# kumar-shridhar/PyTorch-BayesianCNN

Measured on AMD Instinct MI355X. Metric: MC-forward samples/sec, BayesianAlexNet CIFAR-10 bs=512 num_ens=10, higher is better.
Workload: dtype f32; 1 GPU; BayesianAlexNet 3x32x32 -> 10, layer_type=bbb, softplus, bs=512, num_ens=10, forward only; global_batch=512, num_ens_total=10, parallelism=single, launch=hipGraph replay, 2 lane(s) x 4 steps per launch

## Files before the change

include/bbb_hip.h:

```cpp
#ifndef BBB_HIP_H
#define BBB_HIP_H

#include <stdint.h>

#ifdef __cplusplus
extern "C" {
#endif

#define BBB_ABI_VERSION 13
#define BBB_MAX_SEGMENTS 16

#define BBB_EINVAL (-1)
#define BBB_EALIGN (-2)
#define BBB_ESHAPE (-3)

typedef struct bbb_segment {
    const float* mu;
    const float* rho;
    float* w;
    float* sigma;
    const float* eps;
    int64_t n;
    int64_t draw_stride;
    uint32_t stream_id;
// ... 28 lines not shown
    int64_t n;
} bbb_adam_segment_t;

int bbb_adam_step(const bbb_adam_segment_t* segs, int nseg, double lr, double beta1, double beta2, double eps,
                  int64_t step, const float* step_dev, const float* lr_dev, void* stream);

int bbb_eps_dump(float* out, int64_t n, int64_t start, uint64_t seed, uint32_t call, uint32_t stream_id, void* stream);

typedef struct bbb_conv_desc {
    int32_t batch;
    int32_t cin, h, w;
    int32_t cout, kh, kw;
    int32_t stride_h, stride_w, pad_h, pad_w, dil_h, dil_w;
    int32_t draws;
    int64_t x_draw_stride;
    int64_t w_draw_stride;
    int64_t b_draw_stride;
    int32_t act;
    int32_t unit_div;
    int32_t unit_off;
    int32_t x_unit_mod;
    int32_t w_row_pitch;
    int32_t b_offset;
    int32_t x_unit_div;
    int32_t x_unit_off;
    int32_t pool;
    int32_t w_tap_major;
} bbb_conv_desc_t;

int bbb_conv2d_fwd(const bbb_conv_desc_t* d, const float* x, const float* w, const float* bias,
                   float* y, void* stream);

int bbb_lrt_conv2d_fwd(const bbb_conv_desc_t* d, const float* x, const float* w_mu, const float* w_var,
                       const float* b_mu, const float* b_var, float* y,
                       float* act_mu_out, float* act_var_out, const float* eps_ext,
                       uint64_t seed, uint32_t call0, uint32_t stream_id, int sample,
                       const uint32_t* call_dev, void* stream);

int bbb_conv2d_chwn_fwd(const bbb_conv_desc_t* d, const float* x, const float* w, const float* bias,
                        float* y, void* stream);
#define BBB_S3_IN  1u
#define BBB_S3_OUT 2u
int bbb_conv2d_chwn_bf16x3_fwd(const bbb_conv_desc_t* d, const void* x, const float* w, const float* bias, void* y, uint32_t flags,
                               void* stream);
int bbb_maxpool_chwn_s3(const void* x, void* y, int64_t slabs, int channels, int h, int w, int batch, int k, int s, void* stream);
int bbb_s3_convert(const void* src, void* dst, int64_t slabs, int64_t n, int to_s3, void* stream);
#define BBB_C8X3_OUT_F32 1u
#define BBB_C8X3_TILE128 2u
#define BBB_C8X3_TILE256 4u
#define BBB_C8X3_POOL 8u
#define BBB_C8X3_NT_SHIFT 4
#define BBB_C8X3_NT_MASK 0x70u
#define BBB_C8X3_ZERO_LEAD_H(n) (((uint32_t)(n) & 15u) << 8)
#define BBB_C8X3_ZERO_LEAD_W(n) (((uint32_t)(n) & 15u) << 12)
#define BBB_C8X3_ZERO_TRAIL_H(n) (((uint32_t)(n) & 15u) << 16)
#define BBB_C8X3_ZERO_TRAIL_W(n) (((uint32_t)(n) & 15u) << 20)
#define BBB_C8X3_ZERO_MASK 0x00FFFF00u
int bbb_conv2d_c8x3_fwd(const bbb_conv_desc_t* d, const void* x, const float* w, const float* bias, void* y, uint32_t flags,
                        void* stream);
int bbb_c8s3_convert(const void* src, void* dst, int64_t slabs, int channels, int64_t positions, int batch, int to_c8s3, void* stream);
int bbb_lrt_conv2d_c8x3_fwd(const bbb_conv_desc_t* d, const void* x, const float* w_mu, const float* w_var, const float* b_mu,
                            const float* b_var, void* y, uint64_t seed, uint32_t call0, uint32_t stream_id, int sample,
                            const uint32_t* call_dev, uint32_t flags, void* stream);
int bbb_maxpool_chwn_s3sq(const void* x, void* y, int64_t slabs, int channels, int h, int w, int batch, int k, int s, void* stream);
int bbb_s2d_c8s3sq(const float* x, void* y, int64_t blocks, int batch, int channels, int h, int w, int k, int stride, int pad, void* stream);
int bbb_s2d_c8s3(const float* x, void* y, int64_t blocks, int batch, int channels, int h, int w, int k, int stride, int pad, void* stream);
int bbb_w_s2d_tap_major(const float* w, float* out, int64_t rows, int channels, int k, int stride, void* stream);
int bbb_w_tap_major(const float* w, float* out, int64_t rows, int cin, int taps, void* stream);
int bbb_lrt_conv2d_chwn_fwd(const bbb_conv_desc_t* d, const float* x, const float* w_mu, const float* w_var,
                            const float* b_mu, const float* b_var, float* y,
                            float* act_mu_out, float* act_var_out, const float* eps_ext,
                            uint64_t seed, uint32_t call0, uint32_t stream_id, int sample,
                            const uint32_t* call_dev, void* stream);

int64_t bbb_conv2d_chwn_splitk_scratch(const bbb_conv_desc_t* d, int lrt, int32_t* k_split);
int bbb_conv2d_chwn_splitk_fwd(const bbb_conv_desc_t* d, const float* x, const float* w, const float* bias, float* y,
                               int k_split, void* scratch, int64_t scratch_bytes, void* stream);
int bbb_lrt_conv2d_chwn_splitk_fwd(const bbb_conv_desc_t* d, const float* x, const float* w_mu, const float* w_var,
                                   const float* b_mu, const float* b_var, float* y,
                                   float* act_mu_out, float* act_var_out, const float* eps_ext,
                                   uint64_t seed, uint32_t call0, uint32_t stream_id, int sample,
                                   const uint32_t* call_dev, int k_split, void* scratch, int64_t scratch_bytes, void* stream);

int bbb_maxpool_chwn(const float* x, float* y, int64_t planes, int h, int w, int batch, int k, int s, void* stream);

int bbb_pool_act_bwd_chwn(const float* g_out, const float* y, float* g_pre, int64_t planes, int h, int w, int batch,
                          int k, int s, int act, int64_t out_plane_pitch, void* stream);

int bbb_lrt_pool_act_bwd_chwn(const float* g_out, const float* y, const float* act_mu, const float* act_var, float* g_mu,
                              float* g_var, int64_t planes, int64_t moment_planes, int h, int w, int batch, int k, int s, int act,
                              int64_t out_plane_pitch, const float* g_out2, const float* x_out, int64_t x_planes, void* stream);

int bbb_lrt_sample_chwn(const float* act_mu, const float* act_var, float* y, int draws, int channels, int pixels, int batch,
                        int b_offset, int act, uint64_t seed, uint32_t call0, uint32_t stream_id, const uint32_t* call_dev,
                        void* stream);

int bbb_lrt_sample_nchw(const float* act_mu, const float* act_var, float* y, int64_t n, int draws, uint64_t seed,
                        uint32_t call0, uint32_t stream_id, const uint32_t* call_dev, void* stream);

#define BBB_BF16_OUT_F32      1u
#define BBB_BF16_W_TAP_MAJOR  2u
#define BBB_BF16_X_C8         4u
#define BBB_BF16_OUT_C8       8u
int bbb_conv2d_chwn_bf16_fwd(const bbb_conv_desc_t* d, const void* x, const void* w, const float* bias, void* y,
                             uint32_t flags, void* stream);
int bbb_maxpool_chwn_bf16(const void* x, void* y, int64_t planes, int h, int w, int batch, int k, int s, void* stream);
int bbb_nchw_to_chwn_bf16(const float* x, void* y, int batch, int64_t plane, void* stream);
int bbb_nchw_to_chwn_bf16_slices(const float* x, void* y, int batch, int64_t plane, int slices, void* stream);

int bbb_mc_tail(const float* logits, int draws, int batch, int classes, int mean_over,
                float* lse_out, void* stream);

int bbb_mc_tail_cb(const float* logits, int draws, int batch, int classes, int mean_over,
                   float* lse_out, void* stream);
int bbb_mc_tail_cb_bwd(const float* logits, const float* lse, const float* g_lse, float* g_logits, int draws, int batch, int classes,
                       int mean_over, void* stream);

int bbb_elbo_cb_fwd(const float* lse, const int64_t* target, const float* kl, float beta, const float* beta_dev, float train_size,
                    int batch, int classes, float* loss_out, void* stream);
int bbb_elbo_cb_bwd(const float* logits, const float* lse, const int64_t* target, const float* g_loss, float beta,
                    const float* beta_dev, float train_size, float* g_logits, float* g_kl, int draws, int batch, int classes,
                    int mean_over, void* stream);

int bbb_mc_tail_units(const float* logits, int units, int slices, int unit_off, int batch_slice, int classes, int mean_over,
                      float* lse_out, void* stream);

int bbb_mc_tail_units_step(const float* logits, int units, int slices, int unit_off, int batch_slice, int classes, int mean_over,
                           float* lse_out, const float* kl_in, float kl_scale, float* kl_out, uint32_t* counter,
                           uint32_t counter_add, void* stream);

int bbb_mc_tail_groups_step(const float* logits, int groups, int draws, int batch, int classes, int mean_over,
                            float* lse_out, const float* kl_in, float kl_scale, float* kl_out, uint32_t* counter,
                            uint32_t counter_add, void* stream);

int bbb_mc_tail_share_step(const float* logits, int slabs, int steps, int draws, int first_off, int batch, int classes,
                           float* lse_out, const float* kl_in, float kl_scale, float* kl_out, uint32_t* counter,
                           uint32_t counter_add, void* stream);

int bbb_uncertainty(const float* logits, int draws, int batch, int classes, int normalized,
                    float* pred, float* epistemic, float* aleatoric, void* stream);

int bbb_transpose2d(const float* in, float* out, int64_t rows, int64_t cols, void* stream);

int bbb_transpose_batched(const float* in, float* out, int rows, int cols, int nb1, int nb2, int64_t in_b1, int64_t in_b2,
                          int64_t in_row, int64_t out_b1, int64_t out_b2, int64_t out_col, void* stream);

int bbb_transpose_sum_batched(const float* in, float* out, int rows, int cols, const int32_t* nb, const int64_t* in_b,
                              const int64_t* out_b, int64_t in_row, int64_t out_col, int nsum, int64_t in_sum, int64_t square_off,
                              void* stream);

int bbb_flip_transpose_w(const float* w, float* out, int64_t draws, int cout, int cin, int khkw, void* stream);
int bbb_flip_transpose_w_pair(const float* w0, const float* w1, float* out, int64_t draws_each, int cout, int cin, int khkw,
                              void* stream);
typedef struct {
    const float* w0;
    const float* w1;
    float* out;
    int64_t draws;
    int32_t cout, cin, khkw, reserved;
} bbb_flip_seg_t;
int bbb_flip_transpose_w_multi(const bbb_flip_seg_t* segs, int n_segs, void* stream);

int bbb_im2col_pbj(const float* x, float* out, const bbb_conv_desc_t* d, void* stream);

int bbb_plane_sum(const float* x, float* out, int64_t outer, int64_t rows, int64_t cols, int64_t row_pitch, int64_t outer_stride,
                  void* stream);
// ... 11 lines not shown
```

pytorch-bayesiancnn_amd/bbb_hip/_lib.py:

```python
import ctypes
import os

import torch

_HERE = os.path.dirname(os.path.abspath(__file__))
LIB_PATH = os.environ.get("BBB_HIP_LIB") or os.path.join(_HERE, "libbbb_hip.so")

ABI_VERSION = 13
MAX_SEGMENTS = 16
SIGMA_SQUARED = 1
KL_TEXTBOOK = 2
GW_MEAN_ONLY = 4

c_void_p, c_int, c_float = ctypes.c_void_p, ctypes.c_int, ctypes.c_float
c_u64, c_u32, c_i64, c_i32 = ctypes.c_uint64, ctypes.c_uint32, ctypes.c_int64, ctypes.c_int32


class Segment(ctypes.Structure):
    _fields_ = [("mu", c_void_p), ("rho", c_void_p), ("w", c_void_p), ("sigma", c_void_p), ("eps", c_void_p),
                ("n", c_i64), ("draw_stride", c_i64), ("stream_id", c_u32), ("w_row_len", c_u32), ("w_taps", c_u32), ("w_tm_cin", c_u32)]


class AdamSegment(ctypes.Structure):
    _fields_ = [("param", c_void_p), ("grad", c_void_p), ("exp_avg", c_void_p), ("exp_avg_sq", c_void_p), ("n", c_i64)]


class FlipSeg(ctypes.Structure):
    _fields_ = [("w0", c_void_p), ("w1", c_void_p), ("out", c_void_p), ("draws", c_i64), ("cout", c_i32), ("cin", c_i32),
                ("khkw", c_i32), ("reserved", c_i32)]


class ConvDesc(ctypes.Structure):
    _fields_ = [("batch", c_i32), ("cin", c_i32), ("h", c_i32), ("w", c_i32), ("cout", c_i32), ("kh", c_i32),
                ("kw", c_i32), ("stride_h", c_i32), ("stride_w", c_i32), ("pad_h", c_i32), ("pad_w", c_i32),
                ("dil_h", c_i32), ("dil_w", c_i32), ("draws", c_i32), ("x_draw_stride", c_i64),
                ("w_draw_stride", c_i64), ("b_draw_stride", c_i64), ("act", c_i32),
                ("unit_div", c_i32), ("unit_off", c_i32), ("x_unit_mod", c_i32), ("w_row_pitch", c_i32), ("b_offset", c_i32),
                ("x_unit_div", c_i32), ("x_unit_off", c_i32), ("pool", c_i32), ("w_tap_major", c_i32)]


_SIGNATURES = {
    "bbb_reparam_kl_fwd": (c_int, [ctypes.POINTER(Segment), c_int, c_int, c_float, c_float, c_u64, c_u32, c_u32,
                                   c_void_p, c_void_p, c_void_p, c_void_p, c_void_p]),
    "bbb_reparam_partials": (c_i64, [ctypes.POINTER(Segment), c_int]),
    "bbb_reparam_kl_bwd": (c_int, [ctypes.POINTER(Segment), c_int, c_int, c_float, c_float, c_u64, c_u32, c_u32,
                                   c_void_p, ctypes.POINTER(c_void_p), ctypes.POINTER(c_void_p), c_void_p, c_void_p]),
    "bbb_adam_step": (c_int, [ctypes.POINTER(AdamSegment), c_int, ctypes.c_double, ctypes.c_double, ctypes.c_double, ctypes.c_double,
                            c_i64, c_void_p, c_void_p, c_void_p]),
    "bbb_eps_dump": (c_int, [c_void_p, c_i64, c_i64, c_u64, c_u32, c_u32, c_void_p]),
    "bbb_conv2d_fwd": (c_int, [ctypes.POINTER(ConvDesc), c_void_p, c_void_p, c_void_p, c_void_p, c_void_p]),
    "bbb_lrt_conv2d_fwd": (c_int, [ctypes.POINTER(ConvDesc), c_void_p, c_void_p, c_void_p, c_void_p, c_void_p, c_void_p,
                                   c_void_p, c_void_p, c_void_p, c_u64, c_u32, c_u32, c_int, c_void_p, c_void_p]),
    "bbb_conv2d_chwn_fwd": (c_int, [ctypes.POINTER(ConvDesc), c_void_p, c_void_p, c_void_p, c_void_p, c_void_p]),
    "bbb_conv2d_chwn_bf16x3_fwd": (c_int, [ctypes.POINTER(ConvDesc), c_void_p, c_void_p, c_void_p, c_void_p, c_u32, c_void_p]),
    "bbb_maxpool_chwn_s3": (c_int, [c_void_p, c_void_p, c_i64, c_int, c_int, c_int, c_int, c_int, c_int, c_void_p]),
    "bbb_s3_convert": (c_int, [c_void_p, c_void_p, c_i64, c_i64, c_int, c_void_p]),
    "bbb_conv2d_c8x3_fwd": (c_int, [ctypes.POINTER(ConvDesc), c_void_p, c_void_p, c_void_p, c_void_p, c_u32, c_void_p]),
    "bbb_c8s3_convert": (c_int, [c_void_p, c_void_p, c_i64, c_int, c_i64, c_int, c_int, c_void_p]),
    "bbb_w_tap_major": (c_int, [c_void_p, c_void_p, c_i64, c_int, c_int, c_void_p]),
    "bbb_s2d_c8s3": (c_int, [c_void_p, c_void_p, c_i64, c_int, c_int, c_int, c_int, c_int, c_int, c_int, c_void_p]),
    "bbb_s2d_c8s3sq": (c_int, [c_void_p, c_void_p, c_i64, c_int, c_int, c_int, c_int, c_int, c_int, c_int, c_void_p]),
    "bbb_lrt_conv2d_c8x3_fwd": (c_int, [ctypes.POINTER(ConvDesc), c_void_p, c_void_p, c_void_p, c_void_p, c_void_p, c_void_p, c_u64, c_u32,
                                        c_u32, c_int, c_void_p, c_u32, c_void_p]),
    "bbb_maxpool_chwn_s3sq": (c_int, [c_void_p, c_void_p, c_i64, c_int, c_int, c_int, c_int, c_int, c_int, c_void_p]),
    "bbb_w_s2d_tap_major": (c_int, [c_void_p, c_void_p, c_i64, c_int, c_int, c_int, c_void_p]),
    "bbb_lrt_conv2d_chwn_fwd": (c_int, [ctypes.POINTER(ConvDesc), c_void_p, c_void_p, c_void_p, c_void_p, c_void_p, c_void_p,
                                        c_void_p, c_void_p, c_void_p, c_u64, c_u32, c_u32, c_int, c_void_p, c_void_p]),
    "bbb_lrt_sample_chwn": (c_int, [c_void_p, c_void_p, c_void_p, c_int, c_int, c_int, c_int, c_int, c_int, c_u64, c_u32, c_u32, c_void_p,
                                  c_void_p]),
    "bbb_lrt_sample_nchw": (c_int, [c_void_p, c_void_p, c_void_p, c_i64, c_int, c_u64, c_u32, c_u32, c_void_p, c_void_p]),
    "bbb_maxpool_chwn": (c_int, [c_void_p, c_void_p, c_i64, c_int, c_int, c_int, c_int, c_int, c_void_p]),
    "bbb_pool_act_bwd_chwn": (c_int, [c_void_p, c_void_p, c_void_p, c_i64, c_int, c_int, c_int, c_int, c_int, c_int, c_i64, c_void_p]),
    "bbb_lrt_pool_act_bwd_chwn": (c_int, [c_void_p, c_void_p, c_void_p, c_void_p, c_void_p, c_void_p, c_i64, c_i64, c_int, c_int, c_int,
                                          c_int, c_int, c_int, c_i64, c_void_p, c_void_p, c_i64, c_void_p]),
    "bbb_conv2d_chwn_bf16_fwd": (c_int, [ctypes.POINTER(ConvDesc), c_void_p, c_void_p, c_void_p, c_void_p, c_u32, c_void_p]),
    "bbb_maxpool_chwn_bf16": (c_int, [c_void_p, c_void_p, c_i64, c_int, c_int, c_int, c_int, c_int, c_void_p]),
    "bbb_nchw_to_chwn_bf16": (c_int, [c_void_p, c_void_p, c_int, c_i64, c_void_p]),
    "bbb_nchw_to_chwn_bf16_slices": (c_int, [c_void_p, c_void_p, c_int, c_i64, c_int, c_void_p]),
    "bbb_mc_tail": (c_int, [c_void_p, c_int, c_int, c_int, c_int, c_void_p, c_void_p]),
    "bbb_mc_tail_cb": (c_int, [c_void_p, c_int, c_int, c_int, c_int, c_void_p, c_void_p]),
    "bbb_mc_tail_cb_bwd": (c_int, [c_void_p, c_void_p, c_void_p, c_void_p, c_int, c_int, c_int, c_int, c_void_p]),
    "bbb_mc_tail_units": (c_int, [c_void_p, c_int, c_int, c_int, c_int, c_int, c_int, c_void_p, c_void_p]),
    "bbb_mc_tail_units_step": (c_int, [c_void_p, c_int, c_int, c_int, c_int, c_int, c_int, c_void_p, c_void_p, c_float, c_void_p, c_void_p,
                                       c_u32, c_void_p]),
    "bbb_mc_tail_groups_step": (c_int, [c_void_p, c_int, c_int, c_int, c_int, c_int, c_void_p, c_void_p, c_float, c_void_p, c_void_p,
                                        c_u32, c_void_p]),
    "bbb_mc_tail_share_step": (c_int, [c_void_p, c_int, c_int, c_int, c_int, c_int, c_int, c_void_p, c_void_p, c_float, c_void_p, c_void_p,
                                       c_u32, c_void_p]),
    "bbb_uncertainty": (c_int, [c_void_p, c_int, c_int, c_int, c_int, c_void_p, c_void_p, c_void_p, c_void_p]),
    "bbb_transpose2d": (c_int, [c_void_p, c_void_p, c_i64, c_i64, c_void_p]),
    "bbb_flip_transpose_w": (c_int, [c_void_p, c_void_p, c_i64, c_int, c_int, c_int, c_void_p]),
    "bbb_flip_transpose_w_multi": (c_int, [ctypes.POINTER(FlipSeg), c_int, c_void_p]),
    "bbb_flip_transpose_w_pair": (c_int, [c_void_p, c_void_p, c_void_p, c_i64, c_int, c_int, c_int, c_void_p]),
    "bbb_elbo_cb_fwd": (c_int, [c_void_p, c_void_p, c_void_p, ctypes.c_float, c_void_p, ctypes.c_float, c_int, c_int, c_void_p, c_void_p]),
    "bbb_elbo_cb_bwd": (c_int, [c_void_p, c_void_p, c_void_p, c_void_p, ctypes.c_float, c_void_p, ctypes.c_float, c_void_p, c_void_p,
                                c_int, c_int, c_int, c_int, c_void_p]),
    "bbb_im2col_pbj": (c_int, [c_void_p, c_void_p, ctypes.POINTER(ConvDesc), c_void_p]),
    "bbb_transpose_batched": (c_int, [c_void_p, c_void_p, c_int, c_int, c_int, c_int, c_i64, c_i64, c_i64, c_i64, c_i64, c_i64, c_void_p]),
    "bbb_transpose_sum_batched": (c_int, [c_void_p, c_void_p, c_int, c_int, ctypes.POINTER(c_i32), ctypes.POINTER(c_i64),
                                          ctypes.POINTER(c_i64), c_i64, c_i64, c_int, c_i64, c_i64, c_void_p]),
    "bbb_conv2d_chwn_splitk_scratch": (c_i64, [ctypes.POINTER(ConvDesc), c_int, ctypes.POINTER(c_i32)]),
    "bbb_conv2d_chwn_splitk_fwd": (c_int, [ctypes.POINTER(ConvDesc), c_void_p, c_void_p, c_void_p, c_void_p, c_int, c_void_p, c_i64,
                                           c_void_p]),
    "bbb_lrt_conv2d_chwn_splitk_fwd": (c_int, [ctypes.POINTER(ConvDesc), c_void_p, c_void_p, c_void_p, c_void_p, c_void_p, c_void_p,
                                               c_void_p, c_void_p, c_void_p, c_u64, c_u32, c_u32, c_int, c_void_p, c_int, c_void_p, c_i64,
                                               c_void_p]),
    "bbb_plane_sum": (c_int, [c_void_p, c_void_p, c_i64, c_i64, c_i64, c_i64, c_i64, c_void_p]),
    "bbb_sum_leading": (c_int, [c_void_p, c_void_p, c_i64, c_i64, c_void_p]),
    "bbb_lrt_glue": (c_int, [c_void_p, c_void_p, c_void_p, c_void_p, c_i64, c_i64, c_int, c_void_p]),
    "bbb_abi_version": (c_int, []),
    "bbb_build_info": (ctypes.c_char_p, []),
}
EXPORTS = tuple(_SIGNATURES)

_lib = None


class BBBHipError(RuntimeError):
    pass


def lib():
    global _lib
    if _lib is None:
        if not os.path.exists(LIB_PATH):
            raise BBBHipError(
                f"{LIB_PATH} not found: the HIP kernels are not built. Run ./build.sh "
                "(or `python -c 'import __graft_entry__ as g; g.build()'`). There is no CPU fallback.")
        h = ctypes.CDLL(LIB_PATH)
        for name, (res, args) in _SIGNATURES.items():
            fn = getattr(h, name)
            fn.restype = res
            fn.argtypes = args
        if h.bbb_abi_version() != ABI_VERSION:
            raise BBBHipError(f"ABI mismatch: library reports {h.bbb_abi_version()}, binding expects {ABI_VERSION}")
        _lib = h
    return _lib


_ERR = {-1: "BBB_EINVAL (bad argument)", -2: "BBB_EALIGN (pointer not 4-byte aligned)", -3: "BBB_ESHAPE (bad geometry)"}


def check(rc, what):
    if rc != 0:
        raise BBBHipError(f"{what} failed: {_ERR.get(rc, 'hipError_t %d' % rc)}")


def ptr(t):
    return 0 if t is None else t.data_ptr()


def require_device(*tensors, dtype=torch.float32):
    for t in tensors:
        if t is None:
            continue
        if not t.is_cuda:
            raise BBBHipError("bbb_hip computes on an MI355X only (tensor is on %s); there is no CPU path. "
                              "Move the module / input to 'cuda'." % t.device)
        if t.dtype != dtype:
            raise BBBHipError(f"bbb_hip expects {dtype} tensors here, got {t.dtype}")


_raw_stream = getattr(torch._C, "_cuda_getCurrentRawStream", None)


def cur_stream(device):
    if _raw_stream is not None and device.index is not None:
        return _raw_stream(device.index)
    return torch.cuda.current_stream(device).cuda_stream


class _NoGuard:
    def __enter__(self):
        return self

    def __exit__(self, *exc):
        return False


_NO_GUARD = _NoGuard()


def on_device(device):
    if device.index is None or torch.cuda.current_device() == device.index:
        return _NO_GUARD
    return torch.cuda.device(device)
```

pytorch-bayesiancnn_amd/bbb_hip/ops.py:

```python
import contextlib
import ctypes
import os
import itertools
import sys
import threading
import types
import weakref

import torch

from . import _lib, rng
from ._lib import Segment, ConvDesc, check, ptr, require_device, cur_stream, on_device

_scratch = {}
_retired = []


_scope_tls = threading.local()
_scope_ids = itertools.count(1)


class scratch_scope:

    def __init__(self, owner=None, token=None):
# ... 148 lines not shown

def _desc(x, w, stride, padding, dilation, draws, x_shared, w_shared, act):
    d = ConvDesc()
    Ex, B, Cin, H, W = x.shape
    Ew, Cout, Cin2, kh, kw = w.shape
    if Cin != Cin2:
        raise _lib.BBBHipError(f"channel mismatch: input has {Cin}, weight expects {Cin2}")
    sh, sw = _pair(stride)
    ph, pw = _pair(padding)
    dh, dw = _pair(dilation)
    d.batch, d.cin, d.h, d.w, d.cout, d.kh, d.kw = B, Cin, H, W, Cout, kh, kw
    d.stride_h, d.stride_w, d.pad_h, d.pad_w, d.dil_h, d.dil_w = sh, sw, ph, pw, dh, dw
    d.draws = draws
    d.x_draw_stride = 0 if x_shared else B * Cin * H * W
    d.w_draw_stride = 0 if w_shared else Cout * Cin * kh * kw
    d.b_draw_stride = 0 if w_shared else Cout
    d.act = ACT_CODE[act]
    ho = (H + 2 * ph - dh * (kh - 1) - 1) // sh + 1
    wo = (W + 2 * pw - dw * (kw - 1) - 1) // sw + 1
    return d, ho, wo


def conv2d_forward(x, w, bias, stride=1, padding=0, dilation=1, act=None):
    require_device(x, w, bias)
    x, w = x.contiguous(), w.contiguous()
    bias = None if bias is None else bias.contiguous()
    E = max(x.shape[0], w.shape[0])
    if x.shape[0] not in (1, E) or w.shape[0] not in (1, E):
        raise _lib.BBBHipError("leading (draw) dims of x and w must be 1 or equal")
    d, ho, wo = _desc(x, w, stride, padding, dilation, E, x.shape[0] == 1 and E > 1, w.shape[0] == 1 and E > 1, act)
    y = torch.empty((E, x.shape[1], w.shape[1], ho, wo), dtype=torch.float32, device=x.device)
    with on_device(x.device):
        check(_lib.lib().bbb_conv2d_fwd(ctypes.byref(d), x.data_ptr(), w.data_ptr(), ptr(bias), y.data_ptr(),
                                        cur_stream(x.device)), "bbb_conv2d_fwd")
    return y


def lrt_conv2d_forward(x, w_mu, w_var, b_mu, b_var, seed, call0, stream_id, stride=1, padding=0, dilation=1,
                       sample=True, eps=None, want_moments=False, act=None):
    require_device(x, w_mu, w_var, b_mu, b_var, eps)
    x = x.contiguous()
    w_mu, w_var = w_mu.contiguous(), w_var.contiguous()
    b_mu = None if b_mu is None else b_mu.contiguous()
    b_var = None if b_var is None else b_var.contiguous()
    E = x.shape[0]
    d, ho, wo = _desc(x, w_mu.unsqueeze(0), stride, padding, dilation, E, False, True, act)
    d.w_draw_stride = 0
    d.b_draw_stride = 0
    shape = (E, x.shape[1], w_mu.shape[0], ho, wo)
    y = torch.empty(shape, dtype=torch.float32, device=x.device)
    am = torch.empty(shape, dtype=torch.float32, device=x.device) if want_moments else None
    av = torch.empty(shape, dtype=torch.float32, device=x.device) if want_moments else None
    if eps is not None:
        eps = eps.contiguous()
        if eps.numel() != y.numel():
            raise _lib.BBBHipError("external eps must have the output's shape")
    with on_device(x.device):
        check(_lib.lib().bbb_lrt_conv2d_fwd(ctypes.byref(d), x.data_ptr(), w_mu.data_ptr(), w_var.data_ptr(), ptr(b_mu),
                                            ptr(b_var), y.data_ptr(), ptr(am), ptr(av), ptr(eps), seed,
                                            call0 & 0xFFFFFFFF, stream_id, 1 if sample else 0, rng.call_dev_ptr(x.device),
                                            cur_stream(x.device)),
              "bbb_lrt_conv2d_fwd")
    return y, am, av


@contextlib.contextmanager
def graph_capture(graph, stream=None):
    import gc
    gc.collect()
    was = gc.isenabled()
    gc.disable()
    try:
        with torch.cuda.graph(graph, stream=stream, capture_error_mode="thread_local"):
            yield
    finally:
        if was:
            gc.enable()


class LaunchConfig:
    FIELDS = ("gemm_mode", "bf16x3_min_workgroups", "s3_min_images", "split_k", "pool_fusion", "pool_fuse_min_items",
              "pool_fuse_imbalance", "launches_overlap", "pool_fuse_min_items_overlapped", "pool_fuse_weight_budget",
              "bf16_pool_fuse_min_rows", "bf16_pool_fuse_min_rows_overlapped", "bf16_c8", "bf16_c8_min_items", "c8x3", "c8x3_s2d",
              "dropin_precision")
    __slots__ = FIELDS

    def __init__(self, **kw):
        self.gemm_mode = "fp32"
        self.bf16x3_min_workgroups = 256
        self.s3_min_images = 2048
        self.split_k = True
        self.pool_fusion = True
        self.pool_fuse_min_items = 1536
        self.pool_fuse_imbalance = 1.07
        self.launches_overlap = False
        self.pool_fuse_min_items_overlapped = 400
        self.pool_fuse_weight_budget = 1 << 20
        self.bf16_pool_fuse_min_rows = 0
        self.bf16_pool_fuse_min_rows_overlapped = 0
        self.bf16_c8 = True
        self.bf16_c8_min_items = 0
        self.dropin_precision = "fp32"
        self.c8x3 = True
        self.c8x3_s2d = True
        for k, v in kw.items():
            setattr(self, k, v)

    def copy(self, **kw):
        c = LaunchConfig(**{k: getattr(self, k) for k in self.FIELDS})
        for k, v in kw.items():
            setattr(c, k, v)
        return c

    def key(self):
        return tuple(getattr(self, k) for k in self.FIELDS)

    def __repr__(self):
        return "LaunchConfig(%s)" % ", ".join("%s=%r" % (k, getattr(self, k)) for k in self.FIELDS)


_default_config = LaunchConfig()
_tls = threading.local()


def current_config():
    st = getattr(_tls, "stack", None)
    return st[-1] if st else _default_config


class use_config:

    def __init__(self, cfg=None, **fields):
        self.cfg, self.fields = cfg, fields

    def __enter__(self):
        base = self.cfg if self.cfg is not None else current_config()
        cfg = base.copy(**self.fields) if self.fields else base
        st = getattr(_tls, "stack", None)
        if st is None:
            st = _tls.stack = []
        st.append(cfg)
        return cfg

    def __exit__(self, *a):
        _tls.stack.pop()
        return False


_split_plans = {}


def _split_scratch(d, lrt, device):
    if not current_config().split_k:
        return 1, None
    pkey = (bytes(d), bool(lrt))
    plan = _split_plans.get(pkey)
    if plan is None:
        ks = ctypes.c_int32(1)
        need = _lib.lib().bbb_conv2d_chwn_splitk_scratch(ctypes.byref(d), 1 if lrt else 0, ctypes.byref(ks))
        plan = _split_plans[pkey] = (ks.value, int(need))
    ks_v, need = plan
    if ks_v <= 1:
        return 1, None
    if need <= 0:
        return ks_v, None
    buf = _grow(_scratch_key(device, "splitk"), max(int(need), 1 << 22),
                lambda m: torch.zeros(m, dtype=torch.uint8, device=device))
    return ks_v, buf


def _apply_units(d, units, x_per_slice):
    if units is None:
        return
    S, off = int(units[0]), int(units[1])
    if S > 1:
        d.unit_div, d.unit_off = S, off % S
        d.x_unit_mod = S if x_per_slice else 0


def _desc_chwn(x, w, stride, padding, dilation, draws, x_shared, w_shared, act):
    Ex, Cin, H, W, B = x.shape
    d, ho, wo = _desc(_Shape((Ex, B, Cin, H, W)), w, stride, padding, dilation, draws, x_shared, w_shared, act)
    d.x_draw_stride = 0 if x_shared else Cin * H * W * B
    return d, ho, wo


class overlapped_launches(use_config):

    def __init__(self, on=True):
        super().__init__(launches_overlap=bool(on))


def pool_fusion_ok(x_shape, w_shape, stride, padding, dilation, draws, pool_module=None, fp32_kernel=False):
    cfg = current_config()
    if not cfg.pool_fusion or (cfg.gemm_mode != "fp32" and not fp32_kernel):
        return False
    key = (tuple(x_shape[-4:]), tuple(w_shape[-4:]), _pair(stride), _pair(padding), _pair(dilation), int(draws), cfg.launches_overlap,
           cfg.pool_fuse_min_items, cfg.pool_fuse_imbalance, cfg.pool_fuse_min_items_overlapped, cfg.pool_fuse_weight_budget,
           None if pool_module is None else (str(pool_module.kernel_size), str(pool_module.stride), str(pool_module.padding),
                                             str(pool_module.dilation), pool_module.ceil_mode,
                                             getattr(pool_module, "return_indices", False)))
    hit = _pool_rule_cache.get(key)
    if hit is None:
        if len(_pool_rule_cache) > 512:
            _pool_rule_cache.clear()
        hit = _pool_rule_cache[key] = _pool_fusion_rule(x_shape, w_shape, stride, padding, dilation, draws, pool_module)
    return hit


_pool_rule_cache = {}


def is_pool_2x2(pool_module):
    pr = lambda v: (v, v) if isinstance(v, int) else tuple(v)
    return not (pr(pool_module.kernel_size) != (2, 2) or pr(pool_module.stride if pool_module.stride is not None else 2) != (2, 2) or
                pr(pool_module.padding) != (0, 0) or pr(pool_module.dilation) != (1, 1) or pool_module.ceil_mode or
                getattr(pool_module, "return_indices", False))


def _pool_fusion_rule(x_shape, w_shape, stride, padding, dilation, draws, pool_module):
    cfg = current_config()
    if pool_module is not None and not is_pool_2x2(pool_module):
        return False
    B = x_shape[-1]
    xm = torch.empty((1,) + tuple(x_shape[-4:]), device="meta")
    wm = torch.empty((1,) + tuple(w_shape[-4:]), device="meta")
    d, ho, wo = _desc_chwn(xm, wm, stride, padding, dilation, int(draws), False, False, None)
    if ho % 2 or wo % 2 or B % 4:
        return False
    ks = ctypes.c_int32(1)
    _lib.lib().bbb_conv2d_chwn_splitk_scratch(ctypes.byref(d), 0, ctypes.byref(ks))
    if ks.value > 1:
        return False
    per_group = (ho // 2) * (wo // 2) * -(-B // 128)
    if max(1, 128 // per_group) * 64 * w_shape[-3] * w_shape[-2] * w_shape[-1] * 4 > cfg.pool_fuse_weight_budget:
        return False
    items = int(draws) * per_group * -(-w_shape[-4] // 64)
    if cfg.launches_overlap:
        return items >= cfg.pool_fuse_min_items_overlapped
    return items >= cfg.pool_fuse_min_items and -(-items // 256) * 256 <= cfg.pool_fuse_imbalance * items


def conv2d_chwn_forward(x, w, bias, stride=1, padding=0, dilation=1, act=None, out=None, units=None, n_units=None,
                        x_per_slice=False, x_div=1, bf16x3=None, x_s3=False, out_s3=False, x_off=0, pool=False, w_tap_major=False):
    require_device(w, bias)
    require_device(x, dtype=torch.bfloat16 if x_s3 else torch.float32)
    x, w = x.contiguous(), w.contiguous()
    bias = None if bias is None else bias.contiguous()
    w_mem = w
    if w_tap_major:
        if x_s3 or out_s3 or bf16x3:
            raise _lib.BBBHipError("w_tap_major: fp32 kernel only")
        bf16x3 = False
        w = _Shape((w.shape[0], w.shape[1], w.shape[4], w.shape[2], w.shape[3]))
    if x_s3:
        if x.dim() != 6 or x.shape[1] != 3 or x.shape[5] % 8:
            raise _lib.BBBHipError("an S3 input is a bf16 tensor [E|1, 3, C, H, W, B] with B % 8 == 0")
        x5 = _Shape((x.shape[0],) + tuple(x.shape[2:]))
    else:
        x5 = x
    if units is not None and units[0] > 1:
        E = int(n_units)
        if x5.shape[0] != (units[0] if x_per_slice else E):
            raise _lib.BBBHipError("work units: x must hold one slab per unit, or one per batch slice with x_per_slice")
        d, ho, wo = _desc_chwn(x5, w, stride, padding, dilation, E, False, False, act)
        _apply_units(d, units, x_per_slice)
    elif int(x_div) > 1:
        E = w.shape[0]
        if not 0 <= int(x_off) < int(x_div) or x5.shape[0] != -(-(E + int(x_off)) // int(x_div)):
            raise _lib.BBBHipError("x_div: x must hold ceil((E + x_off) / x_div) input slabs for the E weight sets")
        d, ho, wo = _desc_chwn(x5, w, stride, padding, dilation, E, False, False, act)
        d.x_unit_div, d.x_unit_off = int(x_div), int(x_off)
    else:
        E = max(x5.shape[0], w.shape[0])
        if x5.shape[0] not in (1, E) or w.shape[0] not in (1, E):
            raise _lib.BBBHipError("leading (draw) dims of x and w must be 1 or equal")
        d, ho, wo = _desc_chwn(x5, w, stride, padding, dilation, E, x5.shape[0] == 1 and E > 1, w.shape[0] == 1 and E > 1, act)
    if x_s3:
        d.x_draw_stride *= 3
    if w_tap_major:
        d.w_tap_major = 1
    B = x5.shape[4]
    if pool:
        if x_s3 or out_s3 or bf16x3 or ho % 2 or wo % 2:
            raise _lib.BBBHipError("pool=True: fp32 kernel only, even output height and width")
        d.pool = 1
        ho, wo = ho // 2, wo // 2
    shape = (E, 3, w.shape[1], ho, wo, B) if out_s3 else (E, w.shape[1], ho, wo, B)
    odt = torch.bfloat16 if out_s3 else torch.float32
    if out_s3 and B % 8:
        raise _lib.BBBHipError("an S3 output needs B % 8 == 0")
    if out is None:
        y = torch.empty(shape, dtype=odt, device=x.device)
    else:
        if out.numel() != E * (3 if out_s3 else 1) * w.shape[1] * ho * wo * B or not out.is_contiguous() or out.dtype != odt:
            raise _lib.BBBHipError("out= must be a contiguous tensor of the output's size and dtype")
        y = out.view(shape)
    with on_device(x.device):
        if x_s3 or out_s3 or (not pool and (bf16x3 if bf16x3 is not None else current_config().gemm_mode == "bf16x3")
                              and E * ho * wo * -(-w.shape[1] // 64) * -(-B // 128) >= current_config().bf16x3_min_workgroups):
            check(_lib.lib().bbb_conv2d_chwn_bf16x3_fwd(ctypes.byref(d), x.data_ptr(), w_mem.data_ptr(), ptr(bias), y.data_ptr(),
                                                        (1 if x_s3 else 0) | (2 if out_s3 else 0), cur_stream(x.device)),
                  "bbb_conv2d_chwn_bf16x3_fwd")
            return y
        ks, scr = _split_scratch(d, False, x.device)
        if ks > 1 and pool:
            raise _lib.BBBHipError("pool=True: this layer's contraction is split (conv + maxpool_chwn instead)")
        if ks > 1:
            check(_lib.lib().bbb_conv2d_chwn_splitk_fwd(ctypes.byref(d), x.data_ptr(), w_mem.data_ptr(), ptr(bias), y.data_ptr(), ks,
                                                        ptr(scr), 0 if scr is None else scr.numel(), cur_stream(x.device)),
                  "bbb_conv2d_chwn_splitk_fwd")
        else:
            check(_lib.lib().bbb_conv2d_chwn_fwd(ctypes.byref(d), x.data_ptr(), w_mem.data_ptr(), ptr(bias), y.data_ptr(),
                                                 cur_stream(x.device)), "bbb_conv2d_chwn_fwd")
    return y


def s3_from_f32(x):
    require_device(x)
    x = x.contiguous()
    n = x.numel() // x.shape[0]
    y = torch.empty((x.shape[0], 3) + tuple(x.shape[1:]), dtype=torch.bfloat16, device=x.device)
    with on_device(x.device):
        check(_lib.lib().bbb_s3_convert(x.data_ptr(), y.data_ptr(), x.shape[0], n, 1, cur_stream(x.device)), "bbb_s3_convert")
    return y


def s3_to_f32(x):
    require_device(x, dtype=torch.bfloat16)
    x = x.contiguous()
    n = x.numel() // (3 * x.shape[0])
    y = torch.empty((x.shape[0],) + tuple(x.shape[2:]), dtype=torch.float32, device=x.device)
    with on_device(x.device):
        check(_lib.lib().bbb_s3_convert(x.data_ptr(), y.data_ptr(), x.shape[0], n, 0, cur_stream(x.device)), "bbb_s3_convert")
    return y


def maxpool_chwn_s3(x, k, s):
    require_device(x, dtype=torch.bfloat16)
    x = x.contiguous()
    E, three, C, H, W, B = x.shape
    ho, wo = (H - k) // s + 1, (W - k) // s + 1
    y = torch.empty((E, 3, C, ho, wo, B), dtype=torch.bfloat16, device=x.device)
    with on_device(x.device):
        check(_lib.lib().bbb_maxpool_chwn_s3(x.data_ptr(), y.data_ptr(), E, C, H, W, B, int(k), int(s), cur_stream(x.device)),
              "bbb_maxpool_chwn_s3")
    return y


def c8s3_from_f32(x, squares=False):
    require_device(x)
    x = x.contiguous()
    E, C, H, W, B = x.shape
    if C % 8:
        raise _lib.BBBHipError("c8 S3 needs a multiple of 8 channels")
    y = torch.empty((E, 6 if squares else 3, C // 8, H, W, B, 8), dtype=torch.bfloat16, device=x.device)
    with on_device(x.device):
        check(_lib.lib().bbb_c8s3_convert(x.data_ptr(), y.data_ptr(), E, C, H * W, B, 2 if squares else 1, cur_stream(x.device)), "bbb_c8s3_convert")
    return y


def c8s3_to_f32(x):
    require_device(x, dtype=torch.bfloat16)
    x = x.contiguous()
    E, planes, CG, H, W, B, eight = x.shape
    y = torch.empty((E, CG * 8, H, W, B), dtype=torch.float32, device=x.device)
    with on_device(x.device):
        check(_lib.lib().bbb_c8s3_convert(x.data_ptr(), y.data_ptr(), E, CG * 8, H * W, B, 3 if planes == 6 else 0, cur_stream(x.device)),
              "bbb_c8s3_convert")
    return y


def w_tap_major(w):
    require_device(w)
    w = w.contiguous()
    E, Cout, Cin, kh, kw = w.shape
    y = torch.empty((E, Cout, kh * kw, Cin), dtype=torch.float32, device=w.device)
    with on_device(w.device):
        check(_lib.lib().bbb_w_tap_major(w.data_ptr(), y.data_ptr(), E * Cout, Cin, kh * kw, cur_stream(w.device)), "bbb_w_tap_major")
    return y


def s2d_geometry(cin, kernel_size, stride, padding, dilation, h, w):
    (kh, kw), (sh, sw), (ph, pw), (dh, dw) = _pair(kernel_size), _pair(stride), _pair(padding), _pair(dilation)
    if kh != kw or sh != sw or ph != pw or (dh, dw) != (1, 1):
        return None
    ho, wo = (h + 2 * ph - kh) // sh + 1, (w + 2 * pw - kw) // sw + 1
# ... 1351 lines not shown
```

Measured before the change: 8.225 million samples/s.

## Add transformed 9-point convolution path for 2x2 3x3 pad-1 conv layers

Adds a dedicated kernel for 3x3, stride-1, pad-1 convolutions on 2x2 feature maps. It first transforms the weights into nine combined sub-matrices (sums and differences of taps). Each sub-GEMM then runs on a pre-summed input tile using fp32 MFMA, and results are accumulated per output pixel. For small launches, the nine transform points are split across workgroups, and a ticket-based last-arriver reduction sums them. This targets the wasted padded taps and small-grid underutilisation of the generic split-K path on tiny maps, at the cost of an extra weight-transform launch per call and an extra partial-sum scratch round trip.

```diff
diff --git a/include/bbb_hip.h b/include/bbb_hip.h
--- a/include/bbb_hip.h
+++ b/include/bbb_hip.h
@@ -134,6 +134,10 @@
                                    uint64_t seed, uint32_t call0, uint32_t stream_id, int sample,
                                    const uint32_t* call_dev, int k_split, void* scratch, int64_t scratch_bytes, void* stream);
 
+int64_t bbb_conv2d_chwn_t9_scratch(const bbb_conv_desc_t* d);
+int bbb_conv2d_chwn_t9_fwd(const bbb_conv_desc_t* d, const float* x, const float* w, const float* bias, float* y,
+                           void* scratch, int64_t scratch_bytes, void* stream);
+
 int bbb_maxpool_chwn(const float* x, float* y, int64_t planes, int h, int w, int batch, int k, int s, void* stream);
 
 int bbb_pool_act_bwd_chwn(const float* g_out, const float* y, float* g_pre, int64_t planes, int h, int w, int batch,
diff --git a/pytorch-bayesiancnn_amd/bbb_hip/_lib.py b/pytorch-bayesiancnn_amd/bbb_hip/_lib.py
--- a/pytorch-bayesiancnn_amd/bbb_hip/_lib.py
+++ b/pytorch-bayesiancnn_amd/bbb_hip/_lib.py
@@ -105,6 +105,8 @@
     "bbb_lrt_conv2d_chwn_splitk_fwd": (c_int, [ctypes.POINTER(ConvDesc), c_void_p, c_void_p, c_void_p, c_void_p, c_void_p, c_void_p,
                                                c_void_p, c_void_p, c_void_p, c_u64, c_u32, c_u32, c_int, c_void_p, c_int, c_void_p, c_i64,
                                                c_void_p]),
+    "bbb_conv2d_chwn_t9_scratch": (c_i64, [ctypes.POINTER(ConvDesc)]),
+    "bbb_conv2d_chwn_t9_fwd": (c_int, [ctypes.POINTER(ConvDesc), c_void_p, c_void_p, c_void_p, c_void_p, c_void_p, c_i64, c_void_p]),
     "bbb_plane_sum": (c_int, [c_void_p, c_void_p, c_i64, c_i64, c_i64, c_i64, c_i64, c_void_p]),
     "bbb_sum_leading": (c_int, [c_void_p, c_void_p, c_i64, c_i64, c_void_p]),
     "bbb_lrt_glue": (c_int, [c_void_p, c_void_p, c_void_p, c_void_p, c_i64, c_i64, c_int, c_void_p]),
diff --git a/pytorch-bayesiancnn_amd/bbb_hip/ops.py b/pytorch-bayesiancnn_amd/bbb_hip/ops.py
--- a/pytorch-bayesiancnn_amd/bbb_hip/ops.py
+++ b/pytorch-bayesiancnn_amd/bbb_hip/ops.py
@@ -254,7 +254,7 @@
     FIELDS = ("gemm_mode", "bf16x3_min_workgroups", "s3_min_images", "split_k", "pool_fusion", "pool_fuse_min_items",
               "pool_fuse_imbalance", "launches_overlap", "pool_fuse_min_items_overlapped", "pool_fuse_weight_budget",
               "bf16_pool_fuse_min_rows", "bf16_pool_fuse_min_rows_overlapped", "bf16_c8", "bf16_c8_min_items", "c8x3", "c8x3_s2d",
-              "dropin_precision")
+              "dropin_precision", "small_map_transform")
     __slots__ = FIELDS
 
     def __init__(self, **kw):
@@ -262,6 +262,7 @@
         self.bf16x3_min_workgroups = 256
         self.s3_min_images = 2048
         self.split_k = True
+        self.small_map_transform = True
         self.pool_fusion = True
         self.pool_fuse_min_items = 1536
         self.pool_fuse_imbalance = 1.07
@@ -339,6 +340,20 @@
     buf = _grow(_scratch_key(device, "splitk"), max(int(need), 1 << 22),
                 lambda m: torch.zeros(m, dtype=torch.uint8, device=device))
     return ks_v, buf
+
+
+def _t9_scratch(d, device):
+    cfg = current_config()
+    if not (cfg.split_k and cfg.small_map_transform):
+        return None
+    if (d.h, d.w, d.kh, d.kw, d.stride_h, d.stride_w, d.pad_h, d.pad_w, d.dil_h, d.dil_w) != (2, 2, 3, 3, 1, 1, 1, 1, 1, 1):
+        return None
+    if d.pool or d.w_tap_major or d.w_row_pitch:
+        return None
+    need = int(_lib.lib().bbb_conv2d_chwn_t9_scratch(ctypes.byref(d)))
+    if need <= 0:
+        raise _lib.BBBHipError("bbb_conv2d_chwn_t9_scratch: the launch's geometry is not admitted")
+    return _grow(_scratch_key(device, "t9"), max(need, 1 << 22), lambda m: torch.zeros(m, dtype=torch.uint8, device=device))
 
 
 def _apply_units(d, units, x_per_slice):
@@ -475,6 +490,11 @@
                                                         (1 if x_s3 else 0) | (2 if out_s3 else 0), cur_stream(x.device)),
                   "bbb_conv2d_chwn_bf16x3_fwd")
             return y
+        t9 = _t9_scratch(d, x.device)
+        if t9 is not None:
+            check(_lib.lib().bbb_conv2d_chwn_t9_fwd(ctypes.byref(d), x.data_ptr(), w_mem.data_ptr(), ptr(bias), y.data_ptr(),
+                                                    t9.data_ptr(), t9.numel(), cur_stream(x.device)), "bbb_conv2d_chwn_t9_fwd")
+            return y
         ks, scr = _split_scratch(d, False, x.device)
         if ks > 1 and pool:
             raise _lib.BBBHipError("pool=True: this layer's contraction is split (conv + maxpool_chwn instead)")
diff --git a/pytorch-bayesiancnn_amd/csrc/pconv_t9.hip b/pytorch-bayesiancnn_amd/csrc/pconv_t9.hip
--- /dev/null
+++ b/pytorch-bayesiancnn_amd/csrc/pconv_t9.hip
@@ -0,0 +1,396 @@
+#include <hip/hip_runtime.h>
+#include <stdint.h>
+
+#include "../../include/bbb_hip.h"
+#include "bbb_common.cuh"
+
+namespace {
+
+typedef float f32x16 __attribute__((ext_vector_type(16)));
+typedef float f32x4 __attribute__((ext_vector_type(4)));
+typedef uint32_t u32x4 __attribute__((ext_vector_type(4)));
+
+constexpr int kThreads = 256;
+constexpr int BM = 64, BN = 64, BK = 32;
+constexpr int LDW = BN + 1, LDX = BM + 4;
+constexpr int XL = BM / 4;
+constexpr int XRPP = kThreads / XL;
+constexpr int XPASS = BK / XRPP;
+constexpr int kPoints = 9;
+constexpr int kTile = BN * BM;
+constexpr int64_t kTicketBytes = 16384;
+constexpr uint32_t kOOB = 0xFFFFFFF0u;
+constexpr int kS = 0, kA = 1, kB = 2;
+
+#ifndef PCONV_T9_SPLIT_MAX
+#define PCONV_T9_SPLIT_MAX 384
+#endif
+
+struct T9Args {
+    const float* x;
+    const float* wt;
+    const float* bias;
+    float* y;
+    int64_t x_ds, wt_ds, b_ds, y_ds;
+    int32_t B, Cin, Cout, act;
+    int32_t Ntiles, nbt, G, per_xcd;
+    int32_t unit_div, unit_off, x_mod, x_div, x_off;
+    int32_t* tickets;
+    float* part;
+};
+
+__host__ __device__ constexpr int axis_mask(int code) { return code == kS ? 3 : code == kA ? 2 : 1; }
+__host__ __device__ constexpr bool feeds(int o, int pix) {
+    return ((axis_mask(o / 3) >> (pix >> 1)) & 1) && ((axis_mask(o % 3) >> (pix & 1)) & 1);
+}
+
+__device__ __forceinline__ float agpr_read(float a) {
+    float v;
+    asm volatile("v_accvgpr_read_b32 %0, %1" : "=v"(v) : "a"(a));
+    return v;
+}
+__device__ __forceinline__ void agpr_write(float& a, float v) { asm volatile("v_accvgpr_write_b32 %0, %1" : "=a"(a) : "v"(v)); }
+
+__device__ __forceinline__ float tw(int code, float t0, float t1, float t2) { return code == kS ? t1 : code == kA ? t0 - t1 : t2 - t1; }
+
+__global__ __launch_bounds__(256) void t9_weights_kernel(const float* __restrict__ w, float* __restrict__ wt, int64_t pairs, int64_t total,
+                                                         int64_t w_ds) {
+    const int64_t i = (int64_t)blockIdx.x * blockDim.x + threadIdx.x;
+    if (i >= total) return;
+    const int64_t s = i / pairs, pr = i - s * pairs;
+    const float* src = w + s * w_ds + pr * 9;
+    float v[9];
+#pragma unroll
+    for (int k = 0; k < 9; ++k) v[k] = src[k];
+    float* dst = wt + s * kPoints * pairs + pr;
+#pragma unroll
+    for (int o = 0; o < kPoints; ++o) {
+        const int r = o / 3, c = o % 3;
+        const float c0 = tw(c, v[0], v[1], v[2]), c1 = tw(c, v[3], v[4], v[5]), c2 = tw(c, v[6], v[7], v[8]);
+        dst[o * pairs] = tw(r, c0, c1, c2);
+    }
+}
+
+template <bool SPLIT>
+__device__ __forceinline__ void t9_item(const T9Args& p, const int64_t item, const int o_first) {
+    __shared__ __attribute__((aligned(16))) float Xs[BK * LDX];
+    __shared__ float Ws[BK * LDW];
+
+    const int g = (int)(item / p.nbt);
+    const int j = (int)(item - (int64_t)g * p.nbt);
+    const int e = g / p.Ntiles;
+    const int ue = p.unit_off + e;
+    const int ew = p.unit_div > 1 ? ue / p.unit_div : e;
+    const int ex = p.x_div > 1 ? (e + p.x_off) / p.x_div : (p.x_mod > 0 ? ue % p.x_mod : e);
+    const int n0 = (g - e * p.Ntiles) * BN;
+    const int b0 = j * BM;
+
+    const int tid = threadIdx.x;
+    const int lane = tid & 63;
+    const int wave = __builtin_amdgcn_readfirstlane(tid >> 6);
+    const int wn = (wave >> 1) * 32, wm = (wave & 1) * 32;
+    const int lrow = lane & 31, lk = lane >> 5;
+
+    const int64_t x_bytes = (int64_t)p.Cin * 4 * p.B * 4;
+    const int64_t wt_bytes = (int64_t)kPoints * p.Cout * p.Cin * 4;
+    const __amdgpu_buffer_rsrc_t xrs = __builtin_amdgcn_make_buffer_rsrc(const_cast<float*>(p.x + (int64_t)ex * p.x_ds), 0, (int)x_bytes, 0x00020000);
+    const __amdgpu_buffer_rsrc_t wrs = __builtin_amdgcn_make_buffer_rsrc(const_cast<float*>(p.wt + (int64_t)ew * p.wt_ds), 0, (int)wt_bytes, 0x00020000);
+
+    const int wkl = tid & 31, wnl = tid >> 5;
+    const int xb4 = (tid % XL) * 4, xkr = tid / XL;
+    const uint32_t xcol = (uint32_t)(b0 + xb4) * 4u;
+    const uint32_t xrow = (uint32_t)p.B * 4u;
+    const int ntiles = (p.Cin + BK - 1) / BK;
+
+    float wreg[8];
+    f32x4 xreg[XPASS][4];
+    uint32_t wpo = 0;
+    int nsrc = 1;
+    uint32_t xd[4] = {0, 0, 0, 0};
+
+    auto load_tile = [&](int t) {
+        const int ciw = t * BK + wkl;
+#pragma unroll
+        for (int ps = 0; ps < 8; ++ps) {
+            const uint32_t off = ciw < p.Cin ? wpo + ((uint32_t)(n0 + wnl + ps * 8) * (uint32_t)p.Cin + (uint32_t)ciw) * 4u : kOOB;
+            wreg[ps] = __builtin_bit_cast(float, __builtin_amdgcn_raw_buffer_load_b32(wrs, off, 0, 0));
+        }
+#pragma unroll
+        for (int ps = 0; ps < XPASS; ++ps) {
+            const int ci = t * BK + xkr + ps * XRPP;
+            const bool ok = ci < p.Cin;
+            const uint32_t base = (uint32_t)ci * 4u * xrow + xcol;
+#pragma unroll
+            for (int s = 0; s < 4; ++s) {
+                if (s < nsrc) xreg[ps][s] = __builtin_bit_cast(f32x4, __builtin_amdgcn_raw_buffer_load_b128(xrs, ok ? base + xd[s] : kOOB, 0, 0));
+            }
+        }
+    };
+    auto store_tile = [&]() {
+#pragma unroll
+        for (int ps = 0; ps < 8; ++ps) Ws[wkl * LDW + wnl + ps * 8] = wreg[ps];
+#pragma unroll
+        for (int ps = 0; ps < XPASS; ++ps) {
+            f32x4 v = xreg[ps][0];
+            if (nsrc == 2) v = xreg[ps][0] + xreg[ps][1];
+            else if (nsrc == 4) v = (xreg[ps][0] + xreg[ps][1]) + (xreg[ps][2] + xreg[ps][3]);
+            *reinterpret_cast<f32x4*>(&Xs[(xkr + ps * XRPP) * LDX + xb4]) = v;
+        }
+    };
+
+    f32x16 acc;
+    float tot[SPLIT ? 1 : 4][16];
+#pragma unroll
+    for (int r = 0; r < 16; ++r) {
+        acc[r] = 0.0f;
+        if constexpr (!SPLIT) {
+#pragma unroll
+            for (int px = 0; px < 4; ++px) agpr_write(tot[px][r], 0.0f);
+        }
+    }
+
+    constexpr int PD = 4;
+    auto mma_tile = [&]() {
+        float ra[PD + 1], rb[PD + 1];
+        auto fetch = [&](int kk, int slot) {
+            const int krow = kk * 2 + lk;
+            rb[slot] = Xs[krow * LDX + wm + lrow];
+            ra[slot] = Ws[krow * LDW + wn + lrow];
+        };
+#pragma unroll
+        for (int i = 0; i < PD; ++i) fetch(i, i);
+#pragma unroll
+        for (int kk = 0; kk < BK / 2; ++kk) {
+            if (kk + PD < BK / 2) fetch(kk + PD, (kk + PD) % (PD + 1));
+            const int s = kk % (PD + 1);
+            acc = __builtin_amdgcn_mfma_f32_32x32x2f32(ra[s], rb[s], acc, 0, 0, 0);
+            __builtin_amdgcn_sched_barrier(0);
+        }
+    };
+
+    const int o_end = SPLIT ? o_first + 1 : kPoints;
+#pragma clang loop unroll(disable)
+    for (int o = o_first; o < o_end; ++o) {
+        const int rc = o / 3, cc = o - 3 * rc;
+        wpo = (uint32_t)o * (uint32_t)p.Cout * (uint32_t)p.Cin * 4u;
+        {
+            const int h0 = rc == kB ? 1 : 0, w0 = cc == kB ? 1 : 0;
+            const bool two_h = rc == kS, two_w = cc == kS;
+            const uint32_t d00 = (uint32_t)(h0 * 2 + w0) * xrow;
+            nsrc = (two_h ? 2 : 1) * (two_w ? 2 : 1);
+            xd[0] = d00;
+            xd[1] = two_w ? d00 + xrow : d00 + 2 * xrow;
+            xd[2] = d00 + 2 * xrow;
+            xd[3] = d00 + 3 * xrow;
+        }
+        load_tile(0);
+        store_tile();
+        __syncthreads();
+#pragma clang loop unroll(disable)
+        for (int t = 0; t < ntiles; ++t) {
+            const bool more = t + 1 < ntiles;
+            if (more) load_tile(t + 1);
+            mma_tile();
+            __syncthreads();
+            if (more) store_tile();
+            __syncthreads();
+        }
+        if constexpr (!SPLIT) {
+#pragma unroll
+            for (int px = 0; px < 4; ++px) {
+                const bool f = ((axis_mask(rc) >> (px >> 1)) & 1) && ((axis_mask(cc) >> (px & 1)) & 1);
+                if (f) {
+#pragma unroll
+                    for (int r = 0; r < 16; ++r) agpr_write(tot[px][r], agpr_read(tot[px][r]) + acc[r]);
+                }
+            }
+#pragma unroll
+            for (int r = 0; r < 16; ++r) acc[r] = 0.0f;
+        }
+    }
+
+    const int HoWo = 4;
+    constexpr int TW = (BK * LDX) / 1024 >= 4 ? 4 : 2;
+    float* const T = &Xs[(wave % TW) * 1024];
+    if constexpr (SPLIT) {
+        __shared__ int s_last;
+        const __amdgpu_buffer_rsrc_t prs = __builtin_amdgcn_make_buffer_rsrc(p.part + item * kPoints * kTile, 0, kPoints * kTile * 4, 0x00020000);
+#pragma unroll
+        for (int pass = 0; pass < 4 / TW; ++pass) {
+            if ((wave / TW) == pass) {
+#pragma unroll
+                for (int r = 0; r < 16; ++r) T[((r & 3) + 8 * (r >> 2) + 4 * lk) * 32 + lrow] = acc[r];
+#pragma unroll
+                for (int i = 0; i < 4; ++i) {
+                    const int nl = (lane >> 3) + 8 * i, b4 = (lane & 7) * 4;
+                    const f32x4 v4 = *reinterpret_cast<const f32x4*>(&T[nl * 32 + b4]);
+                    const uint32_t off = (uint32_t)((o_first * 64 + wn + nl) * BM + wm + b4) * 4u;
+                    __builtin_amdgcn_raw_buffer_store_b128(__builtin_bit_cast(u32x4, v4), prs, off, 0, 16);
+                }
+            }
+            if (TW < 4) __syncthreads();
+        }
+        asm volatile("s_waitcnt vmcnt(0)" ::: "memory");
+        __syncthreads();
+        if (tid == 0) {
+            const int old = __hip_atomic_fetch_add(p.tickets + item, 1, __ATOMIC_RELAXED, __HIP_MEMORY_SCOPE_AGENT);
+            s_last = old == kPoints - 1;
+            if (old == kPoints - 1) __hip_atomic_store(p.tickets + item, 0, __ATOMIC_RELAXED, __HIP_MEMORY_SCOPE_AGENT);
+        }
+        __syncthreads();
+        if (!s_last) return;
+        const __amdgpu_buffer_rsrc_t yrs = __builtin_amdgcn_make_buffer_rsrc(p.y + (int64_t)e * p.y_ds, 0, (int)((int64_t)p.Cout * HoWo * p.B * 4), 0x00020000);
+        const float* __restrict__ b1g = p.bias ? p.bias + (int64_t)ew * p.b_ds : nullptr;
+#pragma unroll
+        for (int q = 0; q < BM / 16; ++q) {
+            const int f = q * kThreads + tid;
+            const int nl = f / (BM / 4), b4 = (f % (BM / 4)) * 4;
+            const int n = n0 + nl, bb = b0 + b4;
+            const float bn = (b1g && n < p.Cout) ? b1g[n] : 0.0f;
+#pragma unroll
+            for (int px = 0; px < 4; ++px) {
+                f32x4 sum = f32x4{0.0f, 0.0f, 0.0f, 0.0f};
+#pragma unroll
+                for (int o = 0; o < kPoints; ++o) {
+                    if (!feeds(o, px)) continue;
+                    const f32x4 v = __builtin_bit_cast(f32x4, __builtin_amdgcn_raw_buffer_load_b128(prs, (uint32_t)((o * 64 + nl) * BM + b4) * 4u, 0, 16));
+#pragma unroll
+                    for (int c = 0; c < 4; ++c) sum[c] = sum[c] + v[c];
+                }
+                f32x4 out;
+#pragma unroll
+                for (int c = 0; c < 4; ++c) out[c] = bbb::apply_act(sum[c] + bn, p.act);
+                const uint32_t off = ((bb < p.B) & (n < p.Cout)) ? (uint32_t)(((int64_t)n * HoWo + px) * p.B + bb) * 4u : kOOB;
+                __builtin_amdgcn_raw_buffer_store_b128(__builtin_bit_cast(u32x4, out), yrs, off, 0, 0);
+            }
+        }
+        return;
+    } else {
+        const __amdgpu_buffer_rsrc_t brs = __builtin_amdgcn_make_buffer_rsrc(
+            const_cast<float*>(p.bias ? p.bias + (int64_t)ew * p.b_ds : p.x), 0, p.bias ? p.Cout * 4 : 0, 0x00020000);
+        const __amdgpu_buffer_rsrc_t yrs = __builtin_amdgcn_make_buffer_rsrc(p.y + (int64_t)e * p.y_ds, 0, (int)((int64_t)p.Cout * HoWo * p.B * 4), 0x00020000);
+#pragma unroll
+        for (int px = 0; px < 4; ++px) {
+#pragma unroll
+            for (int pass = 0; pass < 4 / TW; ++pass) {
+                if ((wave / TW) == pass) {
+#pragma unroll
+                    for (int r = 0; r < 16; ++r) T[((r & 3) + 8 * (r >> 2) + 4 * lk) * 32 + lrow] = agpr_read(tot[px][r]);
+#pragma unroll
+                    for (int i = 0; i < 4; ++i) {
+                        const int nl = (lane >> 3) + 8 * i, b4 = (lane & 7) * 4;
+                        const int n = n0 + wn + nl, bb = b0 + wm + b4;
+                        const float bn = __builtin_bit_cast(float, __builtin_amdgcn_raw_buffer_load_b32(brs, (uint32_t)n * 4u, 0, 0));
+                        f32x4 v4 = *reinterpret_cast<const f32x4*>(&T[nl * 32 + b4]);
+#pragma unroll
+                        for (int c = 0; c < 4; ++c) v4[c] = bbb::apply_act(v4[c] + bn, p.act);
+                        const uint32_t off = ((bb < p.B) & (n < p.Cout)) ? (uint32_t)(((int64_t)n * HoWo + px) * p.B + bb) * 4u : kOOB;
+                        __builtin_amdgcn_raw_buffer_store_b128(__builtin_bit_cast(u32x4, v4), yrs, off, 0, 0);
+                    }
+                }
+                __syncthreads();
+            }
+        }
+    }
+}
+
+template <bool SPLIT>
+__global__ __launch_bounds__(kThreads) void pconv_t9_kernel(const T9Args p) {
+    const int bid = blockIdx.x;
+    const int xcd = bid & 7;
+    const int64_t blk = (int64_t)xcd * p.per_xcd + (bid >> 3);
+    const int64_t blk_end = (int64_t)(xcd + 1) * p.per_xcd;
+    const int64_t items = (int64_t)p.G * p.nbt;
+    if (blk >= blk_end || blk >= items * (SPLIT ? kPoints : 1)) return;
+    if constexpr (SPLIT) {
+        const int64_t item = blk / kPoints;
+        t9_item<true>(p, item, (int)(blk - item * kPoints));
+    } else {
+        t9_item<false>(p, blk, 0);
+    }
+}
+
+struct T9Plan {
+    int64_t items, nsets, wt_bytes, part_bytes;
+    bool split;
+};
+
+int t9_plan(const bbb_conv_desc_t* d, T9Plan& pl) {
+    if (d == nullptr) return BBB_EINVAL;
+    if (d->batch <= 0 || d->cin <= 0 || d->cout <= 0 || d->draws <= 0 || d->act < 0 || d->act > 2) return BBB_EINVAL;
+    if (d->h != 2 || d->w != 2 || d->kh != 3 || d->kw != 3 || d->stride_h != 1 || d->stride_w != 1 || d->pad_h != 1 || d->pad_w != 1 ||
+        d->dil_h != 1 || d->dil_w != 1)
+        return BBB_EINVAL;
+    if (d->pool != 0 || d->w_tap_major != 0 || d->w_row_pitch != 0) return BBB_EINVAL;
+    if (d->batch % 4 != 0) return BBB_ESHAPE;
+    if (d->x_draw_stride < 0 || d->w_draw_stride < 0 || d->b_draw_stride < 0) return BBB_EINVAL;
+    if (d->unit_div < 0 || d->unit_off < 0 || d->x_unit_mod < 0 || d->b_offset < 0) return BBB_EINVAL;
+    if (d->unit_div > 1 && d->unit_off >= d->unit_div) return BBB_EINVAL;
+    if (d->x_unit_mod > 0 && d->x_unit_mod != d->unit_div) return BBB_EINVAL;
+    if (d->x_unit_div < 0 || d->x_unit_off < 0 || (d->x_unit_div > 1 && (d->unit_div > 1 || d->x_unit_off >= d->x_unit_div)) ||
+        (d->x_unit_div <= 1 && d->x_unit_off != 0))
+        return BBB_EINVAL;
+    if ((int64_t)d->cin * 4 * d->batch * 4 + 4 * (int64_t)(d->batch + 64) * 4 > 0xFFFE0000LL) return BBB_ESHAPE;
+    if ((int64_t)d->cout * 4 * d->batch * 4 > 0x7FFFFFFFLL) return BBB_ESHAPE;
+    if ((int64_t)kPoints * (d->cout + 64) * d->cin * 4 > 0x7FFFFFF0LL) return BBB_ESHAPE;
+    const int64_t ntl = (d->cout + BN - 1) / BN, nbt = (d->batch + BM - 1) / BM;
+    pl.items = (int64_t)d->draws * ntl * nbt;
+    if (pl.items * kPoints > 0x7fffffffLL - 8) return BBB_ESHAPE;
+    const int64_t last = d->unit_div > 1 ? ((int64_t)d->unit_off + d->draws - 1) / d->unit_div : d->draws - 1;
+    pl.nsets = d->w_draw_stride == 0 ? 1 : last + 1;
+    pl.wt_bytes = (pl.nsets * kPoints * d->cout * d->cin * 4 + 255) / 256 * 256;
+    pl.split = pl.items <= PCONV_T9_SPLIT_MAX;
+    pl.part_bytes = pl.split ? pl.items * kPoints * kTile * 4 : 0;
+    return 0;
+}
+
+}
+
+extern "C" int64_t bbb_conv2d_chwn_t9_scratch(const bbb_conv_desc_t* d) {
+    T9Plan pl;
+    if (t9_plan(d, pl) != 0) return 0;
+    return kTicketBytes + pl.wt_bytes + pl.part_bytes;
+}
+
+extern "C" int bbb_conv2d_chwn_t9_fwd(const bbb_conv_desc_t* d, const float* x, const float* w, const float* bias, float* y,
+                                      void* scratch, int64_t scratch_bytes, void* stream) {
+    T9Plan pl;
+    int rc = t9_plan(d, pl);
+    if (rc != 0) return rc;
+    if (x == nullptr || w == nullptr || y == nullptr || scratch == nullptr) return BBB_EINVAL;
+    if ((((uintptr_t)x | (uintptr_t)y) & 15u) != 0 || (((uintptr_t)w | (uintptr_t)bias) & 3u) != 0) return BBB_EALIGN;
+    if ((((uintptr_t)scratch) & 255u) != 0 || scratch_bytes < kTicketBytes + pl.wt_bytes + pl.part_bytes) return BBB_EINVAL;
+    hipStream_t st = (hipStream_t)stream;
+    char* const scr = static_cast<char*>(scratch);
+    float* const wt = reinterpret_cast<float*>(scr + kTicketBytes);
+
+    const int64_t pairs = (int64_t)d->cout * d->cin;
+    const int64_t total = pl.nsets * pairs;
+    const int64_t wblocks = (total + 255) / 256;
+    if (wblocks > 0x7fffffffLL) return BBB_ESHAPE;
+    hipLaunchKernelGGL(t9_weights_kernel, dim3((unsigned)wblocks), dim3(256), 0, st, w, wt, pairs, total, (int64_t)d->w_draw_stride);
+
+    T9Args a = {};
+    a.x = x; a.wt = wt; a.bias = bias; a.y = y;
+    a.x_ds = d->x_draw_stride;
+    a.wt_ds = d->w_draw_stride == 0 ? 0 : kPoints * pairs;
+    a.b_ds = d->b_draw_stride;
+    a.y_ds = (int64_t)d->cout * 4 * d->batch;
+    a.B = d->batch; a.Cin = d->cin; a.Cout = d->cout; a.act = d->act;
+    a.Ntiles = (d->cout + BN - 1) / BN;
+    a.G = a.Ntiles * d->draws;
+    a.nbt = (d->batch + BM - 1) / BM;
+    a.unit_div = d->unit_div; a.unit_off = d->unit_div > 1 ? d->unit_off : 0; a.x_mod = d->x_unit_mod;
+    a.x_div = d->x_unit_div; a.x_off = d->x_unit_off;
+    const int64_t blocks = pl.items * (pl.split ? kPoints : 1);
+    const int64_t per = (blocks + 7) / 8;
+    a.per_xcd = (int32_t)per;
+    if (pl.split) {
+        a.tickets = reinterpret_cast<int32_t*>(scr);
+        a.part = reinterpret_cast<float*>(scr + kTicketBytes + pl.wt_bytes);
+        hipLaunchKernelGGL((pconv_t9_kernel<true>), dim3((unsigned)(8 * per)), dim3(kThreads), 0, st, a);
+    } else {
+        hipLaunchKernelGGL((pconv_t9_kernel<false>), dim3((unsigned)(8 * per)), dim3(kThreads), 0, st, a);
+    }
+    return (int)hipGetLastError();
+}
```

Measured after the change: 8.310 million samples/s, median of 6. +1.0%, better.
